# smoggy-P/gym-Drone2D-ActivePerception

Measured on NVIDIA B200. Metric: env-steps/sec, higher is better.
Workload: dtype f64

## Files before the change

gym_drone2d_activeperception_b200/csrc/d2d_step.cuh:

```cuda
#pragma once
#include "d2d_state.cuh"
#include "d2d_math.cuh"

#if defined(D2D_COLD_NOINLINE) && D2D_COLD_NOINLINE
#define D2D_COLD __noinline__
#else
#define D2D_COLD __forceinline__
#endif

__device__ __forceinline__ uint32_t d2d_smem_u32(const void *p) { return (uint32_t)__cvta_generic_to_shared(p); }
__device__ __forceinline__ void d2d_mbar_init(uint64_t *bar, uint32_t count) {
    asm volatile("mbarrier.init.shared::cta.b64 [%0], %1;" ::"r"(d2d_smem_u32(bar)), "r"(count) : "memory");
    asm volatile("fence.mbarrier_init.release.cluster;" ::: "memory");
}
__device__ __forceinline__ void d2d_mbar_expect_tx(uint64_t *bar, uint32_t bytes) {
    asm volatile("mbarrier.arrive.expect_tx.shared::cta.b64 _, [%0], %1;" ::"r"(d2d_smem_u32(bar)), "r"(bytes) : "memory");
}
__device__ __forceinline__ void d2d_bulk_g2s(void *dst_smem, const void *src_gmem, uint32_t bytes, uint64_t *bar) {
    asm volatile("cp.async.bulk.shared::cluster.global.mbarrier::complete_tx::bytes [%0], [%1], %2, [%3];" ::"r"(
                     d2d_smem_u32(dst_smem)),
                 "l"(src_gmem), "r"(bytes), "r"(d2d_smem_u32(bar))
                 : "memory");
}
__device__ __forceinline__ void d2d_mbar_wait(uint64_t *bar, uint32_t parity) {
// ... 29 lines not shown
};

__host__ __device__ inline size_t d2d_step_smem_bytes(int E, int NP, int HW) {
    size_t b = (size_t)E * D2D_BELIEF_STRIDE + (size_t)E * D2D_GT_ROW_BYTES;
    b += (size_t)E * NP * 8 * 5;
    b += ((size_t)E * NP * 2 + 15) / 16 * 16;
    b += ((size_t)E * HW * 4 + 15) / 16 * 16;
    b = (b + 15) / 16 * 16;
    b += (size_t)E * sizeof(EnvS);
    b += 16 + 16;
    return b;
}

__device__ __forceinline__ BlockCtx d2d_carve(unsigned char *base, int E, int NP, int HW) {
    BlockCtx c;
    size_t o = 0;
    c.belief = base; o += (size_t)E * D2D_BELIEF_STRIDE;
    c.gt = (uint64_t *)(base + o); o += (size_t)E * D2D_GT_ROW_BYTES;
    c.sx = (double *)(base + o); o += (size_t)E * NP * 8;
    c.sy = (double *)(base + o); o += (size_t)E * NP * 8;
    c.sr2 = (double *)(base + o); o += (size_t)E * NP * 8;
    c.mx = (double *)(base + o); o += (size_t)E * NP * 8;
    c.my = (double *)(base + o); o += (size_t)E * NP * 8;
    c.cull = (uint16_t *)(base + o); o += ((size_t)E * NP * 2 + 15) / 16 * 16;
    c.hitw = (uint32_t *)(base + o); o += ((size_t)E * HW * 4 + 15) / 16 * 16;
    o = (o + 15) / 16 * 16;
    c.S = (EnvS *)(base + o); o += (size_t)E * sizeof(EnvS);
    c.mbar = (uint64_t *)(base + o); o += 16;
    c.misc = (int *)(base + o);
    return c;
}

__device__ __forceinline__ void d2d_env_begin(const DevP &P, EnvS &s, bool was_done) {
    const bool rs = s.pending_reset != 0 || (P.auto_reset && was_done);
    s.ox_was_fresh = s.ox_fresh; s.owl_was_fresh = s.owl_fresh;
    s.pending_reset = 0; s.ox_fresh = 0; s.owl_fresh = 0;
    if (rs) {
        s.px = s.p0x; s.py = s.p0y; s.yaw = s.p0yaw; s.vx = 0; s.vy = 0; s.tgx = s.p0x; s.tgy = s.p0y;
        s.steps = 0; s.sm = SM_WAIT_FOR_GOAL; s.fail = 0; s.tcur = 0; s.bufc = 0; s.bufts = 0; s.tracked = 0;
        s.nseg = 0; s.cursor = 0;
        if (P.planner == D2D_PLANNER_JERK) { s.tgx = 0.0; s.tgy = 0.0; }
    }
    s.ix = d2d_cell(s.px, P.scale, P.inv_scale); s.iy = d2d_cell(s.py, P.scale, P.inv_scale);
    s.valid = 1; s.reset = rs; s.jerk_has = 0;
    s.ncull = 0; s.coll_agent = 0; s.arch_cnt = 0; s.arch_ts = 0; s.act_cnt = 0; s.act_ts = 0; s.newly = 0; s.done_now = 0;
}

__device__ D2D_COLD void d2d_load_env_scalars(const DevP &P, EnvS &s, int e) {
    if (e >= P.B) {
        s.valid = 0; s.reset = 0; s.done_now = 0; s.ncull = 0; s.coll_agent = 0;
        return;
    }
    const bool was_done = P.done[e] != 0;
    const uint4 *src = (const uint4 *)(P.rec + e);
    uint4 r[8];
#pragma unroll
    for (int i = 0; i < 8; i++) r[i] = src[i];
#pragma unroll
    for (int i = 0; i < 8; i++) ((uint4 *)&s)[i] = r[i];
    d2d_env_begin(P, s, was_done);
}

__device__ D2D_COLD void d2d_store_env_scalars(const DevP &P, const EnvS &s, int e) {
    uint4 *dst = (uint4 *)(P.rec + e);
#pragma unroll
    for (int i = 0; i < 8; i++) dst[i] = ((const uint4 *)&s)[i];
}

__device__ __forceinline__ void d2d_load_env_warp(const DevP &P, EnvS &s, int e, int lane) {
    unsigned long long w = 0ull;
    uint8_t was_done = 0;
    if (lane < 16) w = ((const unsigned long long *)(P.rec + e))[lane];
    if (lane == 0) was_done = P.done[e];
    if (lane < 16) ((unsigned long long *)&s)[lane] = w;
    __syncwarp();
    if (lane == 0) d2d_env_begin(P, s, was_done != 0);
}
__device__ __forceinline__ void d2d_store_env_warp(const DevP &P, const EnvS &s, int e, int lane) {
    if (lane < 16) ((unsigned long long *)(P.rec + e))[lane] = ((const unsigned long long *)&s)[lane];
}

__device__ __forceinline__ void d2d_issue_bulk(const DevP &P, const BlockCtx &c, int env0, int E, bool want_belief) {
    uint32_t bytes = 0;
    for (int i = 0; i < E; i++) {
        if (!c.S[i].valid) continue;
        bytes += D2D_GT_ROW_BYTES;
        if (want_belief && !c.S[i].reset) bytes += D2D_BELIEF_STRIDE;
    }
    d2d_mbar_expect_tx(c.mbar, bytes);
    for (int i = 0; i < E; i++) {
        if (!c.S[i].valid) continue;
        const size_t e = (size_t)(env0 + i);
        d2d_bulk_g2s(c.gt + (size_t)i * D2D_GRID, P.gt_rows + e * D2D_GRID, D2D_GT_ROW_BYTES, c.mbar);
        if (want_belief && !c.S[i].reset)
            d2d_bulk_g2s(c.belief + (size_t)i * D2D_BELIEF_STRIDE, P.belief + e * D2D_BELIEF_STRIDE, D2D_BELIEF_STRIDE, c.mbar);
    }
}

__device__ D2D_COLD void d2d_reset_arrays(const DevP &P, const BlockCtx &c, int env0, int E, int tid, int T,
                                          uint64_t *early_bulk = nullptr) {
    if (!c.misc[1]) return;
    if (early_bulk) d2d_mbar_wait(early_bulk, 0);
    const int W = D2D_BELIEF_STRIDE / 16;
#pragma unroll 1
    for (int w = tid; w < E * W; w += T) {
        const int i = w / W, o = w - i * W;
        if (!c.S[i].valid || !c.S[i].reset) continue;
        ((uint4 *)(c.belief + (size_t)i * D2D_BELIEF_STRIDE))[o] = uint4{0u, 0u, 0u, 0u};
        ((uint4 *)(P.belief + (size_t)(env0 + i) * D2D_BELIEF_STRIDE))[o] = uint4{0u, 0u, 0u, 0u};
    }
    if (P.rng_key) {
#pragma unroll 1
        for (int w = tid; w < E * 624; w += T) {
            const int i = w / 624, o = w - i * 624;
            if (!c.S[i].valid || !c.S[i].reset) continue;
            const size_t g = (size_t)(env0 + i) * 624 + o;
            P.rng_key[g] = P.rng_key0[g];
            if (o == 0) { const int e2 = env0 + i; P.rng_pos[e2] = P.rng_pos0[e2]; P.rng_has[e2] = P.rng_has0[e2]; P.rng_gauss[e2] = P.rng_gauss0[e2]; }
        }
    }
    if (P.ox_seen) {
        const int W = D2D_OX_SEEN_STRIDE / 2;
#pragma unroll 1
        for (int w = tid; w < E * W; w += T) {
            const int i = w / W, o = w - i * W;
            if (!c.S[i].valid || !c.S[i].reset || c.S[i].ox_was_fresh) continue;
            ((uint32_t *)(P.ox_seen + (size_t)(env0 + i) * D2D_OX_SEEN_STRIDE))[o] = 0u;
            if (o == 0) P.ox_calls[env0 + i] = 0;
        }
    }
    if (P.owl_U) {
#pragma unroll 1
        for (int w = tid; w < E * D2D_OWL_BINS; w += T) {
            const int i = w / D2D_OWL_BINS, o = w - i * D2D_OWL_BINS;
            if (!c.S[i].valid || !c.S[i].reset || c.S[i].owl_was_fresh) continue;
            P.owl_U[(size_t)(env0 + i) * D2D_OWL_BINS + o] = 0.0;
            if (o == 0) P.owl_q[env0 + i] = 0;
        }
    }
}

__device__ __forceinline__ void d2d_reset_prefetch(const DevP &P, const EnvS &s, int e, int lane, double2 &pf_pos,
                                                   double2 &pf_pref) {
    if (s.reset && lane < P.N) {
        const size_t g = (size_t)e * P.NP + lane;
        pf_pos = P.apos0[g]; pf_pref = P.apref0[g];
        asm volatile("prefetch.global.L2 [%0];" ::"l"(P.trk_radius0 + g));
    }
}

template <bool COLLIDE_HERE, bool PF = false>
__device__ __forceinline__ void d2d_phase_agents(const DevP &P, const BlockCtx &c, int env0, int E, int tid, int T,
                                                 double2 pf_pos = double2{0.0, 0.0}, double2 pf_pref = double2{0.0, 0.0},
                                                 double pf_r = 0.0, double2 *keep_pos = nullptr, double2 *keep_pref = nullptr) {
    const double C6 = 0.8660254037844387, S6 = 0.49999999999999994;
    const int N = P.N, NP = P.NP;
#pragma unroll 1
    for (int w = tid; w < E * N; w += T) {
        const int i = w / N, k = w - i * N;
        EnvS &s = c.S[i];
        if (!s.valid) continue;
        const size_t g = (size_t)(env0 + i) * NP + k;
        double2 pos, pref;
        double r;
        if (PF && w == tid) { pos = pf_pos; pref = pf_pref; r = pf_r; }
        else {
            if (s.reset) { pos = P.apos0[g]; pref = P.apref0[g]; }
            else { pos = P.apos[g]; pref = P.apref[g]; }
            r = P.arad[g];
        }
        double vx = pref.x, vy = pref.y;
        const bool rvo = P.motion_rvo != 0;
        if (rvo) {
            const double2 v = P.avel_next[g];
            P.avel[g] = v;
            vx = v.x; vy = v.y;
        }
        const double nx = pos.x + vx * P.dt, ny = pos.y + vy * P.dt;
        bool rebound = false;
        if (d2d_norm2_le(vx, vy, 5.0)) {
            const double qx = D2D_FMA(C6, pref.x, -S6 * pref.y);
            const double qy = D2D_FMA(S6, pref.x, C6 * pref.y);
            pref.x = qx; pref.y = qy;
            rebound = true;
        }
        const double edge = P.scale;
        if (nx < edge + r) pref.x = fabs(pref.x);
        else if (nx > P.map_w - edge - r) pref.x = -fabs(pref.x);
        if (ny < edge + r) pref.y = fabs(pref.y);
        else if (ny > P.map_h - edge - r) pref.y = -fabs(pref.y);
        if (!rebound && !rvo) { vx = pref.x; vy = pref.y; }
        pos.x = pos.x + vx * P.dt;
        pos.y = pos.y + vy * P.dt;
        P.apos[g] = pos;
        P.apref[g] = pref;
        if (PF && keep_pos && w == tid) { *keep_pos = pos; *keep_pref = pref; }
        const int q = i * NP + k;
        c.sx[q] = pos.x; c.sy[q] = pos.y; c.sr2[q] = r * r;
        const double ddx = pos.x - s.px, ddy = pos.y - s.py;
        const double reach = r + P.cull_reach;
        if (ddx * ddx + ddy * ddy <= reach * reach) {
            const int slot = atomicAdd(&s.ncull, 1);
            c.cull[i * NP + slot] = (uint16_t)k;
        }
        if (COLLIDE_HERE) {
            if (d2d_norm2_lt(ddx, ddy, r + P.drone_r)) atomicOr(&s.coll_agent, 1);
        }
    }
}

struct RayOut {
    uint8_t *bel_s;
    int e;
    int patch;
    int wi, wj;
    int border_ok;
    uint32_t *chg;
    int *nchg;
    int defer_mirror;
};
#define D2D_CHG_CAP 64
#define D2D_ACTION_SENTINEL 0x7FF8D2D0AC710F05ull
#define D2D_FUSED_WARP_EXTRA (D2D_CHG_CAP * 4 + 16)

__device__ __forceinline__ void d2d_mark_store(const DevP &P, const RayOut &o, int cell, uint8_t v) {
    o.bel_s[cell] = v;
#if defined(D2D_WARP_PROF) && D2D_WARP_PROF >= 2
    atomicAdd(&P.prof[(size_t)o.e * 12 + 5], 1ull);
#endif
    P.belief[(size_t)o.e * D2D_BELIEF_STRIDE + cell] = v;
    if (o.patch) {
        const int ci = cell / D2D_GRID, cj = cell - ci * D2D_GRID;
        const int u = ci - o.wi, w = cj - o.wj;
        if ((unsigned)u < (unsigned)D2D_LOCAL && (unsigned)w < (unsigned)D2D_LOCAL) {
            const size_t off = (size_t)o.e * D2D_LOCAL_CELLS + u * D2D_LOCAL + w;
            P.local_map[off] = v;
            if (P.lm_mirror && !o.defer_mirror) {
                P.lm_mirror[off] = v;
                atomicAdd((int *)(o.bel_s + D2D_MIRCNT_OFF), 1);
            }
        }
    }
    if (o.chg) {
        const int slot = atomicAdd(o.nchg, 1);
        if (slot < D2D_CHG_CAP) o.chg[slot] = (uint32_t)cell | ((uint32_t)v << 16);
    }
}
__device__ __forceinline__ void d2d_mark(const DevP &P, const RayOut &o, int ci, int cj, uint8_t v) {
    const int cell = ci * D2D_GRID + cj;
    if (o.bel_s[cell] != v) d2d_mark_store(P, o, cell, v);
}

__device__ __forceinline__ double d2d_ray_angle(const DevP &P, double yaw, int ray) {
    const double ray_angle = P.ray_a0 + P.ray_da * (double)ray;
    const double player_angle = D2D_TWO_PI - yaw * D2D_DEG2RAD;
    double a = player_angle + ray_angle;
    a = copysign(d2d_pymod(fabs(a), D2D_TWO_PI), a);
    if (a < 0) a += D2D_TWO_PI;
    return a;
}

template <bool SAFE = false>
__device__ __forceinline__ uint32_t d2d_cast_ray(const DevP &P, const EnvS &s, double a, double slope, const RayOut &o,
                                                 const uint64_t *gt, const double *sx, const double *sy, const double *sr2,
                                                 const uint16_t *cull, uint32_t *hitw) {
    uint32_t hm = 0u;
    const bool faced_right = (a < 90.0 * D2D_DEG2RAD) || (a > 270.0 * D2D_DEG2RAD);
    const bool faced_up = a > D2D_PI;
    const double step = P.scale - 1.0;
    double xs, ys;
    if (fabs(slope) > 1.0) {
        slope = 1.0 / slope;
        ys = faced_up ? -step : step;
        xs = ys * slope;
    } else {
        xs = faced_right ? step : -step;
        ys = xs * slope;
    }
    const double x0 = s.px, y0 = s.py;
    const int nc = s.ncull;
    uint32_t cmask = 0u;
    int mlo = 0x7fff, mhi = -1;
    {
        const double dd2 = xs * xs + ys * ys;
        const float inv_dd2 = 1.0f / (float)dd2;
        const int ncm = nc < 32 ? nc : 32;
#pragma unroll 1
        for (int q = 0; q < ncm; q++) {
            const int k = cull[q];
            const double cx = sx[k] - x0, cy = sy[k] - y0;
            const double cr = cx * ys - cy * xs;
            const double rr = sr2[k] * 1.000001 + 1e-3;
            if (cr * cr <= rr * dd2) {
                cmask |= 1u << q;
                const float t = (float)(cx * xs + cy * ys) * inv_dd2;
                const float hw = sqrtf((float)rr * inv_dd2) + 0.05f;
                mlo = min(mlo, (int)ceilf(t - hw));
                mhi = max(mhi, (int)floorf(t + hw));
            }
        }
        if (nc > 32) { mlo = 0; mhi = 0x7fff; }
    }
    const unsigned mspan = mhi >= mlo ? (unsigned)(mhi - mlo) : 0u;
    if (SAFE) {
        const bool xup = xs > 0.0, yup = ys > 0.0;
        int dcx = xup ? D2D_GRID : -D2D_GRID, dcy = yup ? 1 : -1;
        asm volatile("" : "+r"(dcx), "+r"(dcy));
        const double uxs = fabs(xs), uys = fabs(ys);
        const double ux0 = xup ? x0 : -x0, uy0 = yup ? y0 : -y0;
        double ux = ux0, uy = uy0;
        double uxb = xup ? P.scale * (double)(s.ix + 1) : -(P.scale * (double)s.ix);
        double uyb = yup ? P.scale * (double)(s.iy + 1) : -(P.scale * (double)s.iy);
        const double scale = P.scale;
        const uint32_t bel0 = d2d_smem_u32(o.bel_s);
        uint32_t caddr = bel0 + (uint32_t)(s.ix * D2D_GRID + s.iy);
        int m = 0;
        for (;;) {
            if ((unsigned)(m - mlo) <= mspan) {
                const double x = dcx > 0 ? ux : -ux, y = dcy > 0 ? uy : -uy;
                if (!(0.0 < x && 0.0 < y)) break;
                bool any = false;
                uint32_t mm = cmask;
                while (mm) {
                    const int q = __ffs(mm) - 1;
                    mm &= mm - 1u;
                    const int k = cull[q];
                    const double ex = sx[k] - x, ey = sy[k] - y;
                    if (ex * ex + ey * ey <= sr2[k]) { hm |= 1u << q; any = true; }
                }
#pragma unroll 1
                for (int q = 32; q < nc; q++) {
                    const int k = cull[q];
                    const double ex = sx[k] - x, ey = sy[k] - y;
                    if (ex * ex + ey * ey <= sr2[k]) { atomicOr(&hitw[k >> 5], 1u << (k & 31)); any = true; }
                }
                if (any) break;
            }
            uint32_t bel;
            asm volatile("ld.shared.u8 %0, [%1];" : "=r"(bel) : "r"(caddr));
            if (bel != 2u) {
                if (bel == 1u) break;
                const int cell = (int)(caddr - bel0);
                const int ci = cell / D2D_GRID, cj = cell - ci * D2D_GRID;
                if ((gt[ci] >> cj) & 1ull) {
                    bool in_map = true;
                    if (ci == 0 || cj == 0) {
                        const double x = dcx > 0 ? ux : -ux, y = dcy > 0 ? uy : -uy;
                        in_map = 0.0 < x && 0.0 < y;
                    }
// ... 14 lines not shown
                ".reg .pred pe, pn;\n\t"
                "add.rn.f64 %0, %0, %3;\n\t"
                "setp.lt.s32 pn, %4, 0;\n\t"
                "setp.eq.and.f64 pe, %0, %1, pn;\n\t"
                "setp.lt.or.f64 pe, %0, %1, pe;\n\t"
                "@!pe add.s32 %2, %2, %4;\n\t"
                "@!pe add.rn.f64 %1, %1, %5;\n\t"
                "}" : "+d"(ux), "+d"(uxb), "+r"(caddr) : "d"(uxs), "r"(dcx), "d"(scale));
            asm("{\n\t"
                ".reg .pred pe, pn;\n\t"
                "add.rn.f64 %0, %0, %3;\n\t"
                "setp.lt.s32 pn, %4, 0;\n\t"
                "setp.eq.and.f64 pe, %0, %1, pn;\n\t"
                "setp.lt.or.f64 pe, %0, %1, pe;\n\t"
                "@!pe add.s32 %2, %2, %4;\n\t"
                "@!pe add.rn.f64 %1, %1, %5;\n\t"
                "}" : "+d"(uy), "+d"(uyb), "+r"(caddr) : "d"(uys), "r"(dcy), "d"(scale));
        }
#if defined(D2D_WARP_PROF) && D2D_WARP_PROF >= 2
        atomicAdd(&P.prof[(size_t)o.e * 12 + 6], (unsigned long long)(m + 1));
        atomicMax(&P.prof[(size_t)o.e * 12 + 7], (unsigned long long)(m + 1));
#endif
        return hm;
    }
    int ci = s.ix, cj = s.iy;
    const bool xup = xs > 0.0, yup = ys > 0.0;
    const int sxi = xup ? 1 : -1, syi = yup ? 1 : -1;
    const double uxs = fabs(xs), uys = fabs(ys);
    double ux = xup ? x0 : -x0, uy = yup ? y0 : -y0;
    double uxb = xup ? P.scale * (double)(ci + 1) : -(P.scale * (double)ci);
    double uyb = yup ? P.scale * (double)(cj + 1) : -(P.scale * (double)cj);
    int m = 0;
    for (;;) {
        if ((unsigned)(ci - 1) >= (unsigned)(D2D_GRID - 2) || (unsigned)(cj - 1) >= (unsigned)(D2D_GRID - 2)) {
            const double x = xup ? ux : -ux, y = yup ? uy : -uy;
            if (!(0.0 < x && x < P.map_w && 0.0 < y && y < P.map_h)) break;
        }
        if ((unsigned)(m - mlo) <= mspan) {
            const double x = xup ? ux : -ux, y = yup ? uy : -uy;
            bool any = false;
            uint32_t mm = cmask;
            while (mm) {
                const int q = __ffs(mm) - 1;
                mm &= mm - 1u;
                const int k = cull[q];
                const double ex = sx[k] - x, ey = sy[k] - y;
                if (ex * ex + ey * ey <= sr2[k]) {
                    hm |= 1u << q;
                    any = true;
                }
            }
#pragma unroll 1
            for (int q = 32; q < nc; q++) {
                const int k = cull[q];
                const double ex = sx[k] - x, ey = sy[k] - y;
                if (ex * ex + ey * ey <= sr2[k]) {
                    atomicOr(&hitw[k >> 5], 1u << (k & 31));
                    any = true;
                }
            }
            if (any) break;
        }
        const bool wall = (gt[ci] >> cj) & 1ull;
        bool far = false;
        if (m >= P.m_far) {
            const double fx = ux - (xup ? x0 : -x0), fy = uy - (yup ? y0 : -y0);
            far = (fx * fx + fy * fy) >= P.depth2;
        }
        if (wall || far) {
            if (wall) d2d_mark(P, o, ci, cj, 1);
            break;
        }
        d2d_mark(P, o, ci, cj, 2);
        ux = ux + uxs;
        uy = uy + uys;
        m += 1;
        bool cx = ux >= uxb, cy = uy >= uyb;
        if (ux == uxb || uy == uyb) {
            if (ux == uxb && !xup) cx = false;
            if (uy == uyb && !yup) cy = false;
        }
        if (cx) { ci += sxi; uxb += P.scale; }
        if (cy) { cj += syi; uyb += P.scale; }
    }
    return hm;
}

__device__ __forceinline__ void d2d_publish_hits(uint32_t hm, const uint16_t *cull, uint32_t *hitw) {
    while (hm) {
        const int q = __ffs(hm) - 1;
        hm &= hm - 1u;
        const int k = cull[q];
        atomicOr(&hitw[k >> 5], 1u << (k & 31));
    }
}

__device__ __forceinline__ void d2d_phase_rays(const DevP &P, const BlockCtx &c, int env0, int E, int tid, int T) {
    const int R = P.n_rays, NP = P.NP;
    for (int w = tid; w < E * R; w += T) {
        const int i = w / R, ray = w - i * R;
        const EnvS &s = c.S[i];
        if (!s.valid) continue;
        RayOut o;
        o.bel_s = c.belief + (size_t)i * D2D_BELIEF_STRIDE;
        o.e = env0 + i; o.patch = 0; o.wi = 0; o.wj = 0; o.border_ok = 0; o.chg = nullptr; o.nchg = nullptr; o.defer_mirror = 0;
        const double a = d2d_ray_angle(P, s.yaw, ray);
        const uint32_t hm = d2d_cast_ray(P, s, a, d2d_tan(a), o, c.gt + (size_t)i * D2D_GRID, c.sx + i * NP, c.sy + i * NP,
                                         c.sr2 + i * NP, c.cull + i * NP, c.hitw + i * P.HW);
        d2d_publish_hits(hm, c.cull + i * NP, c.hitw + i * P.HW);
    }
}

__device__ __forceinline__ int d2d_border_intact(const uint64_t *gt, int lane) {
    const uint64_t FULL = (1ull << D2D_GRID) - 1ull, EDGE = 1ull | (1ull << (D2D_GRID - 1));
    bool ok = true;
#pragma unroll
    for (int r = lane; r < D2D_GRID; r += 32) {
        const uint64_t need = (r == 0 || r == D2D_GRID - 1) ? FULL : EDGE;
        ok = ok && ((gt[r] & need) == need);
    }
    return __all_sync(0xffffffffu, ok) ? 1 : 0;
}

template <bool ILP2>
__device__ __forceinline__ void d2d_phase_rays_warp(const DevP &P, const BlockCtx &c, const RayOut &o, int lane) {
    const EnvS &s = c.S[0];
    const int R = P.n_rays;
    uint32_t hm = 0u;
    if (ILP2) {
        for (int r0 = lane; r0 < R; r0 += 64) {
            const int r1 = r0 + 32;
            const double a0 = d2d_ray_angle(P, s.yaw, r0), a1 = d2d_ray_angle(P, s.yaw, r1);
            const double t0 = d2d_tan(a0), t1 = d2d_tan(a1);
            hm |= d2d_cast_ray(P, s, a0, t0, o, c.gt, c.sx, c.sy, c.sr2, c.cull, c.hitw);
            if (r1 < R) hm |= d2d_cast_ray(P, s, a1, t1, o, c.gt, c.sx, c.sy, c.sr2, c.cull, c.hitw);
        }
    } else {
        const bool safe = o.border_ok && (unsigned)s.ix < (unsigned)D2D_GRID && (unsigned)s.iy < (unsigned)D2D_GRID;
#pragma unroll 1
        for (int ray = lane; ray < R; ray += 32) {
            const double a = d2d_ray_angle(P, s.yaw, ray);
            const double tn = d2d_tan(a);
            if (safe) hm |= d2d_cast_ray<true>(P, s, a, tn, o, c.gt, c.sx, c.sy, c.sr2, c.cull, c.hitw);
            else hm |= d2d_cast_ray<false>(P, s, a, tn, o, c.gt, c.sx, c.sy, c.sr2, c.cull, c.hitw);
        }
    }
    hm = __reduce_or_sync(0xffffffffu, hm);
    if ((hm >> lane) & 1u) {
        const int k = c.cull[lane];
        atomicOr(&c.hitw[k >> 5], 1u << (k & 31));
    }
}

struct D2DRng {
    uint32_t *key;
    int pos, has;
    double gauss;
};
__device__ __noinline__ void d2d_mt_regen(uint32_t *mt) {
    const uint32_t UP = 0x80000000u, LO = 0x7fffffffu, MA = 0x9908b0dfu;
    int kk;
    uint32_t y;
#pragma unroll 1
    for (kk = 0; kk < 624 - 397; kk++) { y = (mt[kk] & UP) | (mt[kk + 1] & LO); mt[kk] = mt[kk + 397] ^ (y >> 1) ^ ((y & 1u) ? MA : 0u); }
#pragma unroll 1
    for (; kk < 623; kk++) { y = (mt[kk] & UP) | (mt[kk + 1] & LO); mt[kk] = mt[kk + (397 - 624)] ^ (y >> 1) ^ ((y & 1u) ? MA : 0u); }
    y = (mt[623] & UP) | (mt[0] & LO); mt[623] = mt[396] ^ (y >> 1) ^ ((y & 1u) ? MA : 0u);
}
__device__ __forceinline__ uint32_t d2d_mt_next32(D2DRng &r) {
    if (r.pos == 624) { d2d_mt_regen(r.key); r.pos = 0; }
    uint32_t y = r.key[r.pos++];
    y ^= (y >> 11); y ^= (y << 7) & 0x9d2c5680u; y ^= (y << 15) & 0xefc60000u; y ^= (y >> 18);
    return y;
}
__device__ __forceinline__ double d2d_mt_next_double(D2DRng &r) {
    const int a = (int)(d2d_mt_next32(r) >> 5), b = (int)(d2d_mt_next32(r) >> 6);
    return ((double)a * 67108864.0 + (double)b) / 9007199254740992.0;
}
__device__ __noinline__ double d2d_legacy_gauss(D2DRng &r) {
    if (r.has) { const double t = r.gauss; r.has = 0; r.gauss = 0.0; return t; }
    double f, x1, x2, r2;
    do {
        x1 = 2.0 * d2d_mt_next_double(r) - 1.0;
        x2 = 2.0 * d2d_mt_next_double(r) - 1.0;
        r2 = x1 * x1 + x2 * x2;
    } while (r2 >= 1.0 || r2 == 0.0);
    f = D2D_SQRT(-2.0 * log(r2) / r2);
    r.gauss = f * x1; r.has = 1;
    return f * x2;
}
__device__ __forceinline__ void d2d_measure_env(const DevP &P, const BlockCtx &c, int e) {
    D2DRng r;
    r.key = P.rng_key + (size_t)e * 624; r.pos = P.rng_pos[e]; r.has = P.rng_has[e]; r.gauss = P.rng_gauss[e];
    bool used = false;
#pragma unroll 1
    for (int k = 0; k < P.N; k++) {
        if (!((c.hitw[k >> 5] >> (k & 31)) & 1u)) continue;
        const double g0 = d2d_legacy_gauss(r), g1 = d2d_legacy_gauss(r);
        c.mx[k] = c.sx[k] + P.var_cam * g0;
        c.my[k] = c.sy[k] + P.var_cam * g1;
        used = true;
    }
    if (used) { P.rng_pos[e] = r.pos; P.rng_has[e] = r.has; P.rng_gauss[e] = r.gauss; }
}

__device__ D2D_COLD void d2d_tracker_update(const DevP &P, EnvS &s, size_t g, bool measured, double z0, double z1,
                                            bool was_active) {
    const double q = (P.var_cam != 0.0) ? 0.1 : 0.001;
    double *mu = P.trk_mu + g * 4, *Sg = P.trk_sigma + g * 16;
    bool active = was_active;
    int ts = s.reset ? 1 : P.trk_ts[g];
    if (s.reset) {
        P.trk_radius[g] = P.trk_radius0[g];
        P.trk_active[g] = 0;
        P.trk_ts[g] = 1;
        if (!measured) {
#pragma unroll
            for (int i = 0; i < 4; i++) mu[i] = 0.0;
#pragma unroll
            for (int i = 0; i < 16; i++) Sg[i] = (i == 0 || i == 5) ? 1.0 : ((i == 10 || i == 15) ? 10.0 : 0.0);
        }
    }
    if (!active && !measured) return;
    double m[4], S[16];
    if (active) {
#pragma unroll
        for (int i = 0; i < 4; i++) m[i] = mu[i];
#pragma unroll
        for (int i = 0; i < 16; i++) S[i] = Sg[i];
        m[0] = m[0] + 0.1 * m[2];
        m[1] = m[1] + 0.1 * m[3];
#pragma unroll
        for (int j = 0; j < 4; j++) {
            S[j] = S[j] + 0.1 * S[8 + j];
            S[4 + j] = S[4 + j] + 0.1 * S[12 + j];
        }
#pragma unroll
        for (int i = 0; i < 4; i++) {
            S[4 * i + 0] = S[4 * i + 0] + 0.1 * S[4 * i + 2];
            S[4 * i + 1] = S[4 * i + 1] + 0.1 * S[4 * i + 3];
        }
        S[0] += q; S[5] += q; S[10] += q; S[15] += q;
        ts += 1;
        const double lo = 10.0 + P.agent_radius;
        if (S[0] >= 150.0 || !(lo < m[0] && m[0] < P.map_w - 10.0 - P.agent_radius) ||
            !(lo < m[1] && m[1] < P.map_h - 10.0 - P.agent_radius)) {
            atomicAdd(&s.arch_cnt, 1);
            atomicAdd(&s.arch_ts, ts);
            active = false;
            P.trk_radius[g] = P.agent_radius;
            m[0] = m[1] = m[2] = m[3] = 0.0;
#pragma unroll
            for (int i = 0; i < 16; i++) S[i] = 0.0;
            S[0] = 1.0; S[5] = 1.0; S[10] = 10.0; S[15] = 10.0;
            ts = 1;
        }
        if (measured) {
            const double rz = P.var_cam;
            const double s00 = rz + S[0], s01 = S[1], s10 = S[4], s11 = rz + S[5];
            const double det = s00 * s11 - s01 * s10;
            const double idet = 1.0 / det;
            const double i00 = s11 * idet, i01 = -s01 * idet, i10 = -s10 * idet, i11 = s00 * idet;
            const double r0 = z0 - m[0], r1 = z1 - m[1];
#pragma unroll
            for (int i = 3; i >= 2; i--) {
                const double k0 = S[4 * i] * i00 + S[4 * i + 1] * i10, k1 = S[4 * i] * i01 + S[4 * i + 1] * i11;
                m[i] = m[i] + (k0 * r0 + k1 * r1);
#pragma unroll
                for (int j = 0; j < 4; j++) S[4 * i + j] = ((-k0) * S[j] + (-k1) * S[4 + j]) + S[4 * i + j];
            }
            {
                const double k00 = S[0] * i00 + S[1] * i10, k01 = S[0] * i01 + S[1] * i11;
                const double k10 = S[4] * i00 + S[5] * i10, k11 = S[4] * i01 + S[5] * i11;
                m[0] = m[0] + (k00 * r0 + k01 * r1);
                m[1] = m[1] + (k10 * r0 + k11 * r1);
#pragma unroll
                for (int j = 0; j < 4; j++) {
                    const double a0 = S[j], a1 = S[4 + j];
                    S[j] = (1.0 - k00) * a0 + (-k01) * a1;
                    S[4 + j] = (-k10) * a0 + (1.0 - k11) * a1;
                }
            }
        }
    } else {
        m[0] = z0; m[1] = z1; m[2] = 0.0; m[3] = 0.0;
#pragma unroll
        for (int i = 0; i < 16; i++) S[i] = 0.0;
        S[0] = 1.0; S[5] = 1.0; S[10] = 10.0; S[15] = 10.0;
        ts = 1;
        active = true;
    }
#pragma unroll
    for (int i = 0; i < 4; i++) mu[i] = m[i];
#pragma unroll
    for (int i = 0; i < 16; i++) Sg[i] = S[i];
    P.trk_active[g] = active ? 1 : 0;
    P.trk_ts[g] = ts;
    if (active) {
        atomicAdd(&s.act_cnt, 1);
        atomicAdd(&s.act_ts, ts);
    }
}

template <bool PF = false>
__device__ __forceinline__ void d2d_phase_trackers(const DevP &P, const BlockCtx &c, int env0, int E, int tid, int T,
                                                   uint8_t pf_act = 0) {
// ... 406 lines not shown
    const bool mirror = GATED && P.lm_mirror != nullptr;
    RayOut ro;
    ro.bel_s = c.belief; ro.e = e; ro.patch = patch ? 1 : 0;
    ro.wi = s.ix - 16; ro.wj = s.iy - 16;
    ro.chg = (mirror && patch) ? chg : nullptr; ro.nchg = nchg; ro.defer_mirror = GATED ? 1 : 0;
    D2D_PROF(6);
    d2d_mbar_wait(c.mbar, 0);
    ro.border_ok = d2d_border_intact(c.gt, lane);
    D2D_PROF(1);
    d2d_phase_rays_warp<ILP2>(P, c, ro, lane);
    __syncwarp();
    D2D_PROF(2);
    if (P.var_cam != 0.0) {
        if (lane == 0) d2d_measure_env(P, c, e);
        __syncwarp();
    }
    d2d_phase_trackers<true>(P, c, e, 1, lane, 32, pf_act);
    D2D_PROF(7);
    const int shit = __any_sync(0xffffffffu, lane < 5 ? d2d_static_probe(P, c.gt, s.px, s.py, lane) : 0);
    __syncwarp();
    D2D_PROF(8);
    if (GATED) {
        if (lane == 0) {
            volatile unsigned long long *slot = P.gate + e;
            const long long t0 = clock64();
            unsigned long long bits;
            while ((bits = *slot) == D2D_ACTION_SENTINEL) {
                if (clock64() - t0 > 4000000000ll) { *P.gate_fault = 1u; bits = 0ull; break; }
            }
            action = __longlong_as_double((long long)bits);
            *slot = D2D_ACTION_SENTINEL;
        }
        __syncwarp();
    }
    if (lane == 0) {
        s.tgx = -1.0; s.tgy = -1.0;
        d2d_leader_finish(P, s, c.gt, e, action, true);
        d2d_leader_flags(P, s, c.gt, e, shit);
        if (e == 0) atomicAdd(&P.stats[D2D_STAT_ENV_STEPS], (unsigned long long)P.B);
        if (!GATED && patch && P.lm_mirror) {
            const int nb = *(const int *)(c.belief + D2D_MIRCNT_OFF);
            if (nb) atomicAdd(&P.stats[D2D_STAT_MIRROR_BYTES], (unsigned long long)nb);
        }
    }
    __syncwarp();
    D2D_PROF(9);
    const int n_changed = mirror ? *nchg : 0;
    const bool rewrite = !patch || s.ix != s.obs_ix || s.iy != s.obs_iy || (mirror && n_changed > D2D_CHG_CAP);
    __syncwarp();
    if (rewrite && lane == 0) { s.obs_ix = s.ix; s.obs_iy = s.iy; }
    __syncwarp();
    d2d_store_env_warp(P, s, e, lane);
    if (rewrite) d2d_obs_env_warp(P, c.belief, s.ix, s.iy, e, lane);
    else if (mirror && n_changed > 0) {
        for (int q = lane; q < n_changed; q += 32) {
            const int cell = (int)(chg[q] & 0xFFFFu);
            const int ci = cell / D2D_GRID, cj = cell - ci * D2D_GRID;
            P.lm_mirror[(size_t)e * D2D_LOCAL_CELLS + (ci - ro.wi) * D2D_LOCAL + (cj - ro.wj)] = (uint8_t)(chg[q] >> 16);
        }
        if (lane == 0) atomicAdd(&P.stats[D2D_STAT_MIRROR_BYTES], (unsigned long long)n_changed);
    }
    if (s.done_now) d2d_count_explored_warp(P, c.belief, lane);
    D2D_PROF(3);
}

#define D2D_GATE_STAMP_SLOT(B) ((size_t)(B))

template <int WPB, int MINB, bool SYNC, bool GATED>
__global__ void __launch_bounds__(WPB * 32, MINB) d2d_rollout_warp_kernel(const DevP P, const double *__restrict__ actions,
                                                                          int K, long long action_stride, int sync_every,
                                                                          unsigned int t_first) {
    extern __shared__ __align__(128) unsigned char smem[];
    const int lane = threadIdx.x & 31, wid = threadIdx.x >> 5;
    const int e = blockIdx.x * WPB + wid;
    if (GATED) {
        if (threadIdx.x == 0) *(int *)(smem + (size_t)WPB * d2d_warp_slice_bytes(P.NP, P.HW, D2D_FUSED_WARP_EXTRA)) = 0;
        __syncthreads();
    }
    if (GATED && P.gate_src && blockIdx.x == gridDim.x - 1) {
        unsigned long long &cst = *(unsigned long long *)(smem + (size_t)WPB * d2d_warp_slice_bytes(P.NP, P.HW, D2D_FUSED_WARP_EXTRA) + 128);
        const volatile unsigned long long *hs = (const volatile unsigned long long *)P.gate_stamp_host;
        for (unsigned int t = 0;; t++) {
            if (threadIdx.x == 0) {
                const unsigned long long want = (unsigned long long)(t_first + t);
                const long long t0 = clock64();
                unsigned long long st;
                while ((((st = *hs) >> 1) & 0xffffffffull) != want) {
                    if (clock64() - t0 > 4000000000ll) { *P.gate_fault = 1u; st = (want << 1) | (1ull << 62); break; }
                }
                cst = st;
            }
            __syncthreads();
            const unsigned long long st = cst;
            const bool zero = (st >> 62) & 1ull;
#pragma unroll 1
            for (int i0 = threadIdx.x; i0 < P.B; i0 += 8 * (int)blockDim.x) {
                unsigned long long v[8];
#pragma unroll
                for (int k = 0; k < 8; k++) {
                    const int i = i0 + k * (int)blockDim.x;
                    v[k] = (i < P.B && !zero) ? __ldcv(P.gate_src + i) : 0ull;
                }
#pragma unroll
                for (int k = 0; k < 8; k++) {
                    const int i = i0 + k * (int)blockDim.x;
                    if (i < P.B) P.gate[i] = v[k];
                }
            }
            __syncthreads();
            if (threadIdx.x == 0) {
                __threadfence();
                *(volatile unsigned long long *)(P.gate + D2D_GATE_STAMP_SLOT(P.B)) = st & 0x1ffffffffull;
            }
            if (!(st & 1ull)) return;
        }
    }
    if (e >= P.B) {
        if (SYNC) for (int t = 1; t < K; t++) if (t % sync_every == 0) __syncthreads();
        return;
    }
    unsigned char *slice = smem + (size_t)wid * d2d_warp_slice_bytes(P.NP, P.HW, GATED ? D2D_FUSED_WARP_EXTRA : 0);
    const BlockCtx c = d2d_carve(slice, 1, P.NP, P.HW);
    uint32_t *chg = (uint32_t *)(slice + d2d_step_smem_bytes(1, P.NP, P.HW));
    int *nchg = (int *)(chg + D2D_CHG_CAP);
    unsigned char *blk = smem + (size_t)WPB * d2d_warp_slice_bytes(P.NP, P.HW, GATED ? D2D_FUSED_WARP_EXTRA : 0);
    int *blk_cnt = (int *)blk;
    unsigned int *blk_yaw = (unsigned int *)(blk + 16);
    unsigned int *blk_done = (unsigned int *)(blk + 16 + WPB * 4);
    const int blk_envs = min(WPB, P.B - (int)blockIdx.x * WPB);
    EnvS &s = c.S[0];
    const size_t ga = (size_t)e * P.NP + lane;
    double2 pf_pos = double2{0.0, 0.0}, pf_pref = double2{0.0, 0.0};
    double pf_r = 0.0;
    uint8_t pf_act = 0;
    if (lane < P.N) {
        pf_pos = P.apos[ga]; pf_pref = P.apref[ga]; pf_r = P.arad[ga];
        if (P.trackers) pf_act = P.trk_active[ga];
    }
    double action = GATED ? 0.0 : actions[e];
    if (lane == 0) {
        if (GATED) *nchg = 0;
        d2d_mbar_init(c.mbar, 1);
        d2d_mbar_expect_tx(c.mbar, D2D_GT_ROW_BYTES + D2D_BELIEF_STRIDE);
        d2d_bulk_g2s(c.gt, P.gt_rows + (size_t)e * D2D_GRID, D2D_GT_ROW_BYTES, c.mbar);
        d2d_bulk_g2s(c.belief, P.belief + (size_t)e * D2D_BELIEF_STRIDE, D2D_BELIEF_STRIDE, c.mbar);
        c.misc[0] = 0;
    }
    d2d_load_env_warp(P, s, e, lane);
    if (lane == 0) c.misc[1] = s.reset;
#pragma unroll 1
    for (int w = lane; w < P.HW; w += 32) c.hitw[w] = 0u;
    __syncwarp();
    int border_ok = 0;
    const bool mirror = GATED && P.lm_mirror != nullptr;
#pragma unroll 1
    for (int t = 0;;) {
        D2D_PROF(0);
        d2d_reset_prefetch(P, s, e, lane, pf_pos, pf_pref);
        d2d_reset_arrays(P, c, e, 1, lane, 32, t == 0 ? c.mbar : nullptr);
        d2d_phase_agents<true, true>(P, c, e, 1, lane, 32, pf_pos, pf_pref, pf_r, &pf_pos, &pf_pref);
        if (t == 0 && pf_act && !s.reset) d2d_prefetch_tracker(P, ga);
        if (lane == 0) d2d_leader_begin(P, s);
        __syncwarp();
        const bool refill = s.reset && s.obs_ix == s.ix && s.obs_iy == s.iy && (GATED || P.lm_mirror == nullptr);
        const bool patch = (!s.reset || refill) && s.obs_ix == s.ix && s.obs_iy == s.iy;
        if (refill) d2d_obs_clear_warp(P, e, lane, false);
        RayOut ro;
        ro.bel_s = c.belief; ro.e = e; ro.patch = patch ? 1 : 0;
        ro.wi = s.ix - 16; ro.wj = s.iy - 16;
        ro.chg = (mirror && patch && !refill) ? chg : nullptr; ro.nchg = nchg; ro.defer_mirror = GATED ? 1 : 0;
        if (t == 0) {
            d2d_mbar_wait(c.mbar, 0);
            border_ok = d2d_border_intact(c.gt, lane);
        }
        ro.border_ok = border_ok;
        D2D_PROF(1);
        d2d_phase_rays_warp<false>(P, c, ro, lane);
        __syncwarp();
        D2D_PROF(2);
        if (P.var_cam != 0.0) {
            if (lane == 0) d2d_measure_env(P, c, e);
            __syncwarp();
        }
        d2d_phase_trackers<true>(P, c, e, 1, lane, 32, pf_act);
        const int shit = __any_sync(0xffffffffu, lane < 5 ? d2d_static_probe(P, c.gt, s.px, s.py, lane) : 0);
        __syncwarp();
        int more = (t + 1 < K) ? 1 : 0;
        bool rewrite = false;
        int n_changed = 0;
        if (GATED) {
            if (lane == 0) {
                s.tgx = -1.0; s.tgy = -1.0;
                d2d_leader_finish(P, s, c.gt, e, 0.0, true, false);
                d2d_leader_flags(P, s, c.gt, e, shit, false);
            }
            __syncwarp();
            n_changed = (mirror && !refill) ? *nchg : 0;
            rewrite = !patch || s.ix != s.obs_ix || s.iy != s.obs_iy || (mirror && n_changed > D2D_CHG_CAP);
            __syncwarp();
            if (rewrite && lane == 0) { s.obs_ix = s.ix; s.obs_iy = s.iy; }
            __syncwarp();
            if (rewrite) d2d_obs_env_warp(P, c.belief, s.ix, s.iy, e, lane, false);
            if (s.done_now) d2d_count_explored_warp(P, c.belief, lane);
            D2D_PROF(8);
            if (lane == 0) {
                volatile unsigned long long *slot = P.gate + e;
                volatile unsigned long long *stamp = P.gate + D2D_GATE_STAMP_SLOT(P.B);
                const unsigned long long want = (unsigned long long)(t_first + (unsigned int)t);
                const long long t0 = clock64();
                unsigned long long bits, st = 0ull;
                bool fault = false;
                while ((bits = *slot) == D2D_ACTION_SENTINEL) {
                    if (clock64() - t0 > 4000000000ll) { fault = true; break; }
                }
                if (!fault) {
                    while (((st = *stamp) >> 1) != want) {
                        if (clock64() - t0 > 4000000000ll) { fault = true; break; }
                    }
                }
                if (fault) { *P.gate_fault = 1u; bits = 0ull; st = 0ull; }
                action = __longlong_as_double((long long)bits);
                *slot = D2D_ACTION_SENTINEL;
                more = (int)(st & 1ull);
                s.yaw = d2d_pymod(s.yaw + (action * P.max_yaw_speed) * P.dt, 360.0);
                P.yaw_obs[e] = (float)s.yaw;
            }
            more = __shfl_sync(0xffffffffu, more, 0);
            D2D_PROF(9);
            if (mirror) {
                if (rewrite || refill) {
                    __syncwarp();
                    d2d_obs_mirror_copy_warp(P, e, lane);
                } else if (n_changed > 0) {
                    for (int q = lane; q < n_changed; q += 32) {
                        const int cell = (int)(chg[q] & 0xFFFFu);
                        const int ci = cell / D2D_GRID, cj = cell - ci * D2D_GRID;
                        P.lm_mirror[(size_t)e * D2D_LOCAL_CELLS + (ci - ro.wi) * D2D_LOCAL + (cj - ro.wj)] = (uint8_t)(chg[q] >> 16);
                    }
                    if (lane == 0) atomicAdd(&P.stats[D2D_STAT_MIRROR_BYTES], (unsigned long long)n_changed);
                }
            }
            __syncwarp();
        } else {
            if (lane == 0) {
                s.tgx = -1.0; s.tgy = -1.0;
                d2d_leader_finish(P, s, c.gt, e, action, true);
                d2d_leader_flags(P, s, c.gt, e, shit);
                if (patch && P.lm_mirror) {
                    int *cnt = (int *)(c.belief + D2D_MIRCNT_OFF);
                    const int nb = *cnt;
                    if (nb) { atomicAdd(&P.stats[D2D_STAT_MIRROR_BYTES], (unsigned long long)nb); *cnt = 0; }
                }
            }
            __syncwarp();
            rewrite = !patch || s.ix != s.obs_ix || s.iy != s.obs_iy;
            __syncwarp();
            if (rewrite && lane == 0) { s.obs_ix = s.ix; s.obs_iy = s.iy; }
            __syncwarp();
            if (rewrite) d2d_obs_env_warp(P, c.belief, s.ix, s.iy, e, lane);
            if (s.done_now) d2d_count_explored_warp(P, c.belief, lane);
        }
        D2D_PROF(4);
        if (GATED) {
            int last = 0;
            if (lane == 0) {
                atomicExch(&blk_yaw[wid], __float_as_uint((float)s.yaw)); atomicExch(&blk_done[wid], (unsigned int)s.done_now);
                __threadfence_block();
                last = atomicAdd(blk_cnt, 1) == blk_envs - 1 ? 1 : 0;
            }
            last = __shfl_sync(0xffffffffu, last, 0);
            if (last) {
                __threadfence_block();
                const int e0 = (int)blockIdx.x * WPB;
                if (lane < blk_envs) {
                    if (P.yaw_mirror) P.yaw_mirror[e0 + lane] = __uint_as_float(atomicOr(&blk_yaw[lane], 0u));
                    if (P.done_mirror) P.done_mirror[e0 + lane] = (uint8_t)atomicOr(&blk_done[lane], 0u);
                }
                __syncwarp();
                if (lane == 0) {
                    *blk_cnt = 0;
                    __threadfence();
                    const unsigned long long n = atomicAdd(P.gate_count, (unsigned long long)blk_envs) + (unsigned long long)blk_envs;
                    if (n == (unsigned long long)P.B * (unsigned long long)(t + 1)) {
                        atomicAdd(&P.stats[D2D_STAT_ENV_STEPS], (unsigned long long)P.B);
                        asm volatile("fence.acq_rel.sys;" ::: "memory");
                        *(volatile unsigned int *)P.gate_done = t_first + (unsigned int)t;
                    }
                }
            }
        }
        D2D_PROF(3);
        t += 1;
        if (!more) break;
        if (SYNC && t % sync_every == 0) __syncthreads();
        if (!GATED) action = actions[(size_t)t * (size_t)action_stride + e];
        if (P.trackers && lane < P.N) pf_act = P.trk_active[ga];
#pragma unroll 1
        for (int w = lane; w < P.HW; w += 32) c.hitw[w] = 0u;
        __syncwarp();
        if (lane == 0) {
            const bool was_done = s.done_now != 0;
            d2d_env_begin(P, s, was_done);
            c.misc[1] = s.reset;
            if (GATED) *nchg = 0;
        }
        __syncwarp();
    }
    d2d_store_env_warp(P, s, e, lane);
    if (!GATED && e == 0 && lane == 0) atomicAdd(&P.stats[D2D_STAT_ENV_STEPS], (unsigned long long)P.B * (unsigned long long)K);
}
```

Baseline: 233.0 million.

## March two rays per lane with interleaved DDA and cached static probe

Adds a paired ray caster in which each lane marches two rays in lockstep. Before marching it culls agents against both rays and narrows the step window where agent hit tests run, and it uses inline PTX for the predicated grid-stepping. This is meant to raise instruction-level parallelism and cut per-step agent checks in the ray phase. The step loop also spills the action to shared memory around the ray phase, reloads agent prefetch state from shared/global, and skips the static obstacle probe when the drone has not moved. These add complexity and register pressure, and carry some risk of behavioural divergence from the single-ray path.

```diff
diff --git a/gym_drone2d_activeperception_b200/csrc/d2d_step.cuh b/gym_drone2d_activeperception_b200/csrc/d2d_step.cuh
--- a/gym_drone2d_activeperception_b200/csrc/d2d_step.cuh
+++ b/gym_drone2d_activeperception_b200/csrc/d2d_step.cuh
@@ -205,7 +205,7 @@
 template <bool COLLIDE_HERE, bool PF = false>
 __device__ __forceinline__ void d2d_phase_agents(const DevP &P, const BlockCtx &c, int env0, int E, int tid, int T,
                                                  double2 pf_pos = double2{0.0, 0.0}, double2 pf_pref = double2{0.0, 0.0},
-                                                 double pf_r = 0.0, double2 *keep_pos = nullptr, double2 *keep_pref = nullptr) {
+                                                 double pf_r = 0.0) {
     const double C6 = 0.8660254037844387, S6 = 0.49999999999999994;
     const int N = P.N, NP = P.NP;
 #pragma unroll 1
@@ -247,7 +247,6 @@
         pos.y = pos.y + vy * P.dt;
         P.apos[g] = pos;
         P.apref[g] = pref;
-        if (PF && keep_pos && w == tid) { *keep_pos = pos; *keep_pref = pref; }
         const int q = i * NP + k;
         c.sx[q] = pos.x; c.sy[q] = pos.y; c.sr2[q] = r * r;
         const double ddx = pos.x - s.px, ddy = pos.y - s.py;
@@ -568,6 +567,231 @@
     }
 }
 
+struct D2DMarch {
+    double ux, uy, uxb, uyb, uxs, uys;
+    uint32_t caddr;
+    int dcx, dcy;
+    uint32_t cmask;
+    int mlo;
+    unsigned mspan;
+};
+
+__device__ __forceinline__ int d2d_march_init(const DevP &P, const EnvS &s, double a, double slope, uint32_t bel0,
+                                              D2DMarch &r, double &xs, double &ys) {
+    const bool faced_right = (a < 90.0 * D2D_DEG2RAD) || (a > 270.0 * D2D_DEG2RAD);
+    const bool faced_up = a > D2D_PI;
+    const double step = P.scale - 1.0;
+    if (fabs(slope) > 1.0) {
+        slope = 1.0 / slope;
+        ys = faced_up ? -step : step;
+        xs = ys * slope;
+    } else {
+        xs = faced_right ? step : -step;
+        ys = xs * slope;
+    }
+    const bool xup = xs > 0.0, yup = ys > 0.0;
+    r.dcx = xup ? D2D_GRID : -D2D_GRID; r.dcy = yup ? 1 : -1;
+    r.uxs = fabs(xs); r.uys = fabs(ys);
+    r.ux = xup ? s.px : -s.px; r.uy = yup ? s.py : -s.py;
+    r.uxb = xup ? P.scale * (double)(s.ix + 1) : -(P.scale * (double)s.ix);
+    r.uyb = yup ? P.scale * (double)(s.iy + 1) : -(P.scale * (double)s.iy);
+    r.caddr = bel0 + (uint32_t)(s.ix * D2D_GRID + s.iy);
+    const float q = sqrtf((float)P.depth2 / (float)(xs * xs + ys * ys)) * 0.9999f;
+    return q < 1e9f ? max(P.m_far, (int)q) : P.m_far;
+}
+
+__device__ __forceinline__ void d2d_march_cell(const DevP &P, const D2DMarch &r, uint32_t bel, bool depth, double px, double py,
+                                               const uint64_t *gt, uint32_t bel0, int &cell, uint32_t &v, bool &end) {
+    cell = (int)(r.caddr - bel0);
+    const int ci = cell / D2D_GRID, cj = cell - ci * D2D_GRID;
+    const bool wall = (gt[ci] >> cj) & 1ull;
+    const double fx = r.ux - (r.dcx > 0 ? px : -px), fy = r.uy - (r.dcy > 0 ? py : -py);
+    const bool far = depth && (fx * fx + fy * fy) >= P.depth2;
+    const double x = r.dcx > 0 ? r.ux : -r.ux, y = r.dcy > 0 ? r.uy : -r.uy;
+    const bool in_map = (ci != 0 && cj != 0) || (0.0 < x && 0.0 < y);
+    if (bel == 1u) { v = 0u; end = true; }
+    else if (bel == 2u) { v = 0u; end = far; }
+    else if (wall) { v = in_map ? 1u : 0u; end = true; }
+    else { v = far ? 0u : 2u; end = far; }
+}
+
+__device__ __forceinline__ uint32_t d2d_cast_ray_pair(const DevP &P, const EnvS &s, double aA, double tA, double aB, double tB,
+                                                      bool two, const RayOut &o, const uint64_t *gt, const double *sx,
+                                                      const double *sy, const double *sr2, const uint16_t *cull,
+                                                      uint32_t *hitw) {
+    const uint32_t bel0 = d2d_smem_u32(o.bel_s);
+    D2DMarch A, B;
+    double xsA, ysA, xsB, ysB;
+    const int mf = min(d2d_march_init(P, s, aA, tA, bel0, A, xsA, ysA), d2d_march_init(P, s, aB, tB, bel0, B, xsB, ysB));
+    const int nc = s.ncull;
+    int wlo;
+    unsigned wspan;
+    {
+        const double x0 = s.px, y0 = s.py;
+        const double ddA = xsA * xsA + ysA * ysA, ddB = xsB * xsB + ysB * ysB;
+        const float invA = 1.0f / (float)ddA, invB = 1.0f / (float)ddB;
+        uint32_t cmA = 0u, cmB = 0u;
+        int loA = 0x7fff, hiA = -1, loB = 0x7fff, hiB = -1;
+        const int ncm = nc < 32 ? nc : 32;
+#pragma unroll 1
+        for (int q = 0; q < ncm; q++) {
+            const int k = cull[q];
+            const double cx = sx[k] - x0, cy = sy[k] - y0;
+            const double rr = sr2[k] * 1.000001 + 1e-3;
+            const double crA = cx * ysA - cy * xsA, crB = cx * ysB - cy * xsB;
+            if (crA * crA <= rr * ddA) {
+                cmA |= 1u << q;
+                const float t = (float)(cx * xsA + cy * ysA) * invA;
+                const float hw = sqrtf((float)rr * invA) + 0.05f;
+                loA = min(loA, (int)ceilf(t - hw));
+                hiA = max(hiA, (int)floorf(t + hw));
+            }
+            if (crB * crB <= rr * ddB) {
+                cmB |= 1u << q;
+                const float t = (float)(cx * xsB + cy * ysB) * invB;
+                const float hw = sqrtf((float)rr * invB) + 0.05f;
+                loB = min(loB, (int)ceilf(t - hw));
+                hiB = max(hiB, (int)floorf(t + hw));
+            }
+        }
+        if (nc > 32) { loA = 0; hiA = 0x7fff; loB = 0; hiB = 0x7fff; }
+        A.cmask = cmA; A.mlo = loA; A.mspan = hiA >= loA ? (unsigned)(hiA - loA) : 0u;
+        B.cmask = cmB; B.mlo = loB; B.mspan = hiB >= loB ? (unsigned)(hiB - loB) : 0u;
+        wlo = min(loA, loB);
+        const int whi = max(hiA, hiB);
+        wspan = whi >= wlo ? (unsigned)(whi - wlo) : 0u;
+        wlo -= mf; A.mlo -= mf; B.mlo -= mf;
+    }
+    if (!two) { B.dcx = 0; B.dcy = 0; }
+    asm volatile("" : "+r"(A.dcx), "+r"(A.dcy), "+r"(B.dcx), "+r"(B.dcy));
+    const double scale = P.scale;
+    uint32_t hm = 0u;
+    int n = -mf;
+    auto end_ray = [&](bool b) {
+#if defined(D2D_WARP_PROF) && D2D_WARP_PROF >= 2
+        atomicAdd(&P.prof[(size_t)o.e * 12 + 6], (unsigned long long)(n + mf + 1));
+        atomicMax(&P.prof[(size_t)o.e * 12 + 7], (unsigned long long)(n + mf + 1));
+#endif
+        if (b) { B.dcx = 0; B.dcy = 0; } else { A.dcx = 0; A.dcy = 0; }
+    };
+    for (;;) {
+        uint32_t todo = (unsigned)(n - wlo) <= wspan ? ((A.dcy != 0 && (unsigned)(n - A.mlo) <= A.mspan ? 1u : 0u) |
+                                                         (B.dcy != 0 && (unsigned)(n - B.mlo) <= B.mspan ? 2u : 0u)) : 0u;
+        while (todo) {
+            const bool b = (todo & 1u) == 0u;
+            todo &= todo - 1u;
+            const double ux = b ? B.ux : A.ux, uy = b ? B.uy : A.uy;
+            const double x = (b ? B.dcx : A.dcx) > 0 ? ux : -ux, y = (b ? B.dcy : A.dcy) > 0 ? uy : -uy;
+            bool any = !(0.0 < x && 0.0 < y);
+            if (!any) {
+                uint32_t mm = b ? B.cmask : A.cmask;
+                while (mm) {
+                    const int q = __ffs(mm) - 1;
+                    mm &= mm - 1u;
+                    const int k = cull[q];
+                    const double ex = sx[k] - x, ey = sy[k] - y;
+                    if (ex * ex + ey * ey <= sr2[k]) { hm |= 1u << q; any = true; }
+                }
+#pragma unroll 1
+                for (int q = 32; q < nc; q++) {
+                    const int k = cull[q];
+                    const double ex = sx[k] - x, ey = sy[k] - y;
+                    if (ex * ex + ey * ey <= sr2[k]) { atomicOr(&hitw[k >> 5], 1u << (k & 31)); any = true; }
+                }
+            }
+            if (any) end_ray(b);
+        }
+        uint32_t belA, belB;
+        asm volatile("ld.shared.u8 %0, [%1];" : "=r"(belA) : "r"(A.caddr));
+        asm volatile("ld.shared.u8 %0, [%1];" : "=r"(belB) : "r"(B.caddr));
+        const bool sA = A.dcy != 0 && (belA != 2u || n >= 0);
+        const bool sB = B.dcy != 0 && (belB != 2u || n >= 0);
+        if (sA || sB) {
+            const double px = s.px, py = s.py;
+            int cellA, cellB;
+            uint32_t vA, vB;
+            bool endA, endB;
+            d2d_march_cell(P, A, belA, n >= 0, px, py, gt, bel0, cellA, vA, endA);
+            d2d_march_cell(P, B, belB, n >= 0, px, py, gt, bel0, cellB, vB, endB);
+            uint32_t st = (sA && vA ? 1u : 0u) | (sB && vB ? 2u : 0u);
+            while (st) {
+                const bool b = (st & 1u) == 0u;
+                st &= st - 1u;
+                d2d_mark_store(P, o, b ? cellB : cellA, (uint8_t)(b ? vB : vA));
+            }
+            if (sA && endA) end_ray(false);
+            if (sB && endB) end_ray(true);
+        }
+        if ((A.dcy | B.dcy) == 0) break;
+        n += 1;
+        asm("{\n\t"
+            ".reg .pred pe, pn;\n\t"
+            "add.rn.f64 %0, %0, %3;\n\t"
+            "setp.lt.s32 pn, %4, 0;\n\t"
+            "setp.eq.and.f64 pe, %0, %1, pn;\n\t"
+            "setp.lt.or.f64 pe, %0, %1, pe;\n\t"
+            "@!pe add.s32 %2, %2, %4;\n\t"
+            "@!pe add.rn.f64 %1, %1, %5;\n\t"
+            "}" : "+d"(A.ux), "+d"(A.uxb), "+r"(A.caddr) : "d"(A.uxs), "r"(A.dcx), "d"(scale));
+        asm("{\n\t"
+            ".reg .pred pe, pn;\n\t"
+            "add.rn.f64 %0, %0, %3;\n\t"
+            "setp.lt.s32 pn, %4, 0;\n\t"
+            "setp.eq.and.f64 pe, %0, %1, pn;\n\t"
+            "setp.lt.or.f64 pe, %0, %1, pe;\n\t"
+            "@!pe add.s32 %2, %2, %4;\n\t"
+            "@!pe add.rn.f64 %1, %1, %5;\n\t"
+            "}" : "+d"(B.ux), "+d"(B.uxb), "+r"(B.caddr) : "d"(B.uxs), "r"(B.dcx), "d"(scale));
+        asm("{\n\t"
+            ".reg .pred pe, pn;\n\t"
+            "add.rn.f64 %0, %0, %3;\n\t"
+            "setp.lt.s32 pn, %4, 0;\n\t"
+            "setp.eq.and.f64 pe, %0, %1, pn;\n\t"
+            "setp.lt.or.f64 pe, %0, %1, pe;\n\t"
+            "@!pe add.s32 %2, %2, %4;\n\t"
+            "@!pe add.rn.f64 %1, %1, %5;\n\t"
+            "}" : "+d"(A.uy), "+d"(A.uyb), "+r"(A.caddr) : "d"(A.uys), "r"(A.dcy), "d"(scale));
+        asm("{\n\t"
+            ".reg .pred pe, pn;\n\t"
+            "add.rn.f64 %0, %0, %3;\n\t"
+            "setp.lt.s32 pn, %4, 0;\n\t"
+            "setp.eq.and.f64 pe, %0, %1, pn;\n\t"
+            "setp.lt.or.f64 pe, %0, %1, pe;\n\t"
+            "@!pe add.s32 %2, %2, %4;\n\t"
+            "@!pe add.rn.f64 %1, %1, %5;\n\t"
+            "}" : "+d"(B.uy), "+d"(B.uyb), "+r"(B.caddr) : "d"(B.uys), "r"(B.dcy), "d"(scale));
+    }
+    return hm;
+}
+
+__device__ __forceinline__ void d2d_phase_rays_pair_warp(const DevP &P, const BlockCtx &c, const RayOut &o, int lane) {
+    const EnvS &s = c.S[0];
+    const int R = P.n_rays;
+    uint32_t hm = 0u;
+    const bool safe = o.border_ok && (unsigned)s.ix < (unsigned)D2D_GRID && (unsigned)s.iy < (unsigned)D2D_GRID;
+    if (safe) {
+        const int NPR = (R + 1) >> 1;
+#pragma unroll 1
+        for (int p = lane; p < NPR; p += 32) {
+            const bool two = p + NPR < R;
+            const double aA = d2d_ray_angle(P, s.yaw, p), aB = d2d_ray_angle(P, s.yaw, two ? p + NPR : p);
+            const double tA = d2d_tan(aA), tB = d2d_tan(aB);
+            hm |= d2d_cast_ray_pair(P, s, aA, tA, aB, tB, two, o, c.gt, c.sx, c.sy, c.sr2, c.cull, c.hitw);
+        }
+    } else {
+#pragma unroll 1
+        for (int ray = lane; ray < R; ray += 32) {
+            const double a = d2d_ray_angle(P, s.yaw, ray);
+            hm |= d2d_cast_ray<false>(P, s, a, d2d_tan(a), o, c.gt, c.sx, c.sy, c.sr2, c.cull, c.hitw);
+        }
+    }
+    hm = __reduce_or_sync(0xffffffffu, hm);
+    if ((hm >> lane) & 1u) {
+        const int k = c.cull[lane];
+        atomicOr(&c.hitw[k >> 5], 1u << (k & 31));
+    }
+}
+
 struct D2DRng {
     uint32_t *key;
     int pos, has;
@@ -1280,13 +1504,15 @@
     for (int w = lane; w < P.HW; w += 32) c.hitw[w] = 0u;
     __syncwarp();
     int border_ok = 0;
+    int shit = 0;
+    bool probe_stale = true;
     const bool mirror = GATED && P.lm_mirror != nullptr;
 #pragma unroll 1
     for (int t = 0;;) {
         D2D_PROF(0);
         d2d_reset_prefetch(P, s, e, lane, pf_pos, pf_pref);
         d2d_reset_arrays(P, c, e, 1, lane, 32, t == 0 ? c.mbar : nullptr);
-        d2d_phase_agents<true, true>(P, c, e, 1, lane, 32, pf_pos, pf_pref, pf_r, &pf_pos, &pf_pref);
+        d2d_phase_agents<true, true>(P, c, e, 1, lane, 32, pf_pos, pf_pref, pf_r);
         if (t == 0 && pf_act && !s.reset) d2d_prefetch_tracker(P, ga);
         if (lane == 0) d2d_leader_begin(P, s);
         __syncwarp();
@@ -1302,16 +1528,21 @@
             border_ok = d2d_border_intact(c.gt, lane);
         }
         ro.border_ok = border_ok;
+        if (!GATED && lane == 0) *(double *)(c.misc + 2) = action;
         D2D_PROF(1);
-        d2d_phase_rays_warp<false>(P, c, ro, lane);
+        d2d_phase_rays_pair_warp(P, c, ro, lane);
         __syncwarp();
+        if (!GATED) action = *(const double *)(c.misc + 2);
+        pf_pos = double2{0.0, 0.0}; pf_pref = double2{0.0, 0.0}; pf_r = 0.0;
+        if (lane < P.N) { pf_pos = double2{c.sx[lane], c.sy[lane]}; pf_pref = P.apref[ga]; pf_r = P.arad[ga]; }
         D2D_PROF(2);
         if (P.var_cam != 0.0) {
             if (lane == 0) d2d_measure_env(P, c, e);
             __syncwarp();
         }
         d2d_phase_trackers<true>(P, c, e, 1, lane, 32, pf_act);
-        const int shit = __any_sync(0xffffffffu, lane < 5 ? d2d_static_probe(P, c.gt, s.px, s.py, lane) : 0);
+        if (probe_stale || s.reset) shit = __any_sync(0xffffffffu, lane < 5 ? d2d_static_probe(P, c.gt, s.px, s.py, lane) : 0);
+        probe_stale = s.nseg != 0;
         __syncwarp();
         int more = (t + 1 < K) ? 1 : 0;
         bool rewrite = false;
```

Result: faster. 235.9 million (median of 6 runs) (+1.2%).
